# 360CVGroup/PlanGen

Hardware: AMD Instinct MI355X
Metric: images/sec, 384px layout2image (576 image tokens, CFG, VQ-16 decode), bs=64 per MI355X (higher is better)
Workload: dtype bf16

## Files before the change

plangen_amd/csrc/attn_decode.h:

```cpp
#pragma once
#include <type_traits>
#include "kernels.h"

template <int NV>
__device__ __forceinline__ void sum_slabs(const float* __restrict__ p, long slab, int S, const int (&offs)[NV], float (&acc)[NV]) {
    for (int s0 = 0; s0 < S; s0 += 4) {
        float t[4][NV];
#pragma unroll
        for (int u = 0; u < 4; ++u) {
            const float* q = p + (long)(s0 + u < S ? s0 + u : S - 1) * slab;
#pragma unroll
            for (int v = 0; v < NV; ++v) t[u][v] = q[offs[v]];
        }
#pragma unroll
        for (int u = 0; u < 4; ++u)
            if (s0 + u < S) {
#pragma unroll
                for (int v = 0; v < NV; ++v) acc[v] += t[u][v];
            }
    }
}

template <typename T, int UN, int NW, int ABL = 0>
__global__ __launch_bounds__(64 * NW) void attn_decode_fused_kernel(const int32_t* __restrict__ row_order, const int32_t* __restrict__ len_p,
                                                              const int32_t* __restrict__ n_dec_p, T* __restrict__ kc, T* __restrict__ vc,
                                                              int nh, int slots, int shared_len, int shared_row,
                                                              const float* __restrict__ qkv, long slab, T* __restrict__ obuf,
                                                              const float* __restrict__ cos_t, const float* __restrict__ sin_t,
                                                              const int32_t* __restrict__ pos_off_p, int S, int max_pos, float scale) {
    constexpr int EPV = ET<T>::EPV, LPK = 128 / EPV, KPI = 64 / LPK, NST = NW * KPI;
    __shared__ float s_o[NST][128];
    __shared__ float s_m[NST], s_l[NST];
    __shared__ __attribute__((aligned(16))) float s_q[128];
    __shared__ float s_k[128], s_v[128];
    __shared__ float s_new;
    constexpr int NIT = (ABL & 32) ? 2 : 1;
    const int tid = threadIdx.x, w = tid >> 6, l = tid & 63;
    const int head = blockIdx.x;
// ... 24 lines not shown
            kv[u] = NTL ? __builtin_nontemporal_load((const u32x4*)(kb + (long)key * 128)) : *(const u32x4*)(kb + (long)key * 128);
        }
#pragma unroll
        for (int u = 0; u < UN; ++u) {
            int key = base + u * KPI + grp;
            key = key < k1 ? key : k1 - 1;
            key = key < 0 ? 0 : key;
            vv[u] = NTL ? __builtin_nontemporal_load((const u32x4*)(vb + (long)key * 128)) : *(const u32x4*)(vb + (long)key * 128);
        }
    };
    const int seg_k1 = sh ? kstart : nprev;
    const int base0 = w * KPW;
    const bool have0 = base0 < seg_k1;
    const int o6[6] = {0, 64, HD, HD + 64, 2 * HD, 2 * HD + 64};
    float t4[4][6], cs = 0.f, sn = 0.f;
    int pos = pos_off_p[row] + slot;
    if (pos >= max_pos) pos = max_pos - 1;
    const float* const qrow = qkv + (long)row * 3 * HD + head * 128 + (tid & 63);
    if (tid < 64) {
        if constexpr (ABL & 2) {
#pragma unroll
            for (int u = 0; u < 4; ++u)
#pragma unroll
                for (int v = 0; v < 6; ++v) t4[u][v] = 0.01f * (float)(tid + v);
            cs = 1.f; sn = 0.f;
        } else {
#pragma unroll
        for (int u = 0; u < 4; ++u) {
            const float* qq = qrow + (long)(u < S ? u : S - 1) * slab;
#pragma unroll
            for (int v = 0; v < 6; ++v) t4[u][v] = qq[o6[v]];
        }
        cs = cos_t[(long)pos * 64 + tid]; sn = sin_t[(long)pos * 64 + tid];
        }
    }
    __builtin_amdgcn_sched_barrier(0);
    if (sh) issue(kshr, vshr, base0, seg_k1, std::false_type{}); else issue(kpriv, vpriv, base0, seg_k1, std::true_type{});
    __builtin_amdgcn_sched_barrier(0);

    if (tid < 64) {
        const int j = tid;
        float a6[6] = {0.f, 0.f, 0.f, 0.f, 0.f, 0.f};
#pragma unroll
        for (int u = 0; u < 4; ++u)
#pragma unroll
            for (int v = 0; v < 6; ++v) asm volatile("" : "+v"(t4[u][v])::"memory");
#pragma unroll
        for (int u = 0; u < 4; ++u)
            if (u < S) {
#pragma unroll
                for (int v = 0; v < 6; ++v) a6[v] += t4[u][v];
            }
        if (S > 4) sum_slabs<6>(qrow + 4 * slab, slab, S - 4, o6, a6);
        const float q0 = a6[0], q1 = a6[1], k0 = a6[2], k1 = a6[3], v0 = a6[4], v1 = a6[5];
        const float c = cs;
// ... 125 lines not shown
    __syncthreads();
    if (tid < 128) {
        float Mx = s_new;
#pragma unroll
        for (int i = 0; i < NST; ++i) Mx = fmaxf(Mx, s_m[i]);
        const float fn = __expf(s_new - Mx);
        float num = fn * s_v[tid], den = fn;
#pragma unroll
        for (int i = 0; i < NST; ++i) {
            const float f = (s_m[i] > -INFINITY) ? __expf(s_m[i] - Mx) : 0.f;
            num = fmaf(f, s_o[i][tid], num);
            den = fmaf(f, s_l[i], den);
        }
        ET<T>::st(obuf + (long)row * HD + head * 128 + tid, num / den);
    }
    if (!(ABL & 1) && tid < 64 && slot < slots) {
        const float* src = (l < 32 ? s_k : s_v) + (l & 31) * 4;
        T* dst = (l < 32 ? kc : vc) + cbase + (long)slot * 128 + (l & 31) * 4;
        if constexpr (sizeof(T) == 2) {
            u32x2 pk; pk.x = pack_bf16x2(src[0], src[1]); pk.y = pack_bf16x2(src[2], src[3]);
            *(u32x2*)dst = pk;
        } else {
            *(f32x4*)dst = *(const f32x4*)src;
        }
    }
    if constexpr (NIT > 1) __syncthreads();
    }
}
```

plangen_amd/csrc/diag_api.hip:

```cpp
#include "engine.h"
#include "diag.h"

extern "C" {

int pg_diag_set_option(pg_handle h, const char* key, int64_t value) {
    if (!h || !key) return PG_ERR_ARG;
    h->tune.diag = diag_hooks();
    if (!strcmp(key, "skip_attn")) { h->skip_attn = value != 0; return PG_OK; }
    if (!strcmp(key, "attn_variant")) { h->tune.attn_variant = (int)value; h->tune_epoch++; return PG_OK; }
    if (!strcmp(key, "attn_waves")) { h->tune.attn_waves = (int)value; h->tune_epoch++; return PG_OK; }
    if (!strcmp(key, "split_target_small")) { h->tune.split_small = (int)value; h->tune_epoch++; return PG_OK; }
    if (!strcmp(key, "split_target_mid")) { h->tune.split_mid = (int)value; h->tune_epoch++; return PG_OK; }
    if (!strcmp(key, "gn_epilogue256")) { h->tune.gn_epilogue256 = value != 0; return PG_OK; }
    if (!strcmp(key, "defer_norm")) { h->defer_norm = value != 0; h->tune_epoch++; return PG_OK; }
    if (!strcmp(key, "fuse_rope")) { h->fuse_rope = value != 0; h->tune_epoch++; return PG_OK; }
    if (!strcmp(key, "force_swiglu")) { h->force_swiglu = value != 0; h->tune_epoch++; return PG_OK; }
    if (!strcmp(key, "lpt_order")) { h->lpt_order = value != 0; h->tune_epoch++; return PG_OK; }
    h->err = std::string("unknown diagnostics option ") + key;
    return PG_ERR_ARG;
}

}
```

plangen_amd/csrc/diag_ops.hip:

```cpp
#include <type_traits>
#include <vector>
#include "kernels.h"
#include "diag.h"
#include "../../include/plangen_hip.h"

namespace {
struct LocalTune {
    PgTune t;
    const PgTune* saved;
    LocalTune() : saved(pg_tune) { t.diag = nullptr; pg_tune = &t; }
    ~LocalTune() { pg_tune = saved; }
};
constexpr int kMaxGridYZ = 65535;
bool to_host(std::vector<int32_t>& dst, const int32_t* src, int n) {
    dst.assign(n > 0 ? n : 0, 0);
    if (n <= 0) return true;
    if (!src) return false;
    return hipMemcpy(dst.data(), src, (size_t)n * 4, hipMemcpyDeviceToHost) == hipSuccess;
}
int launched(hipStream_t s) { (void)s; return hipGetLastError() == hipSuccess ? PG_OK : PG_ERR_HIP; }
}

extern "C" {

// ... 30 lines not shown
    }
    void* q = qbuf;
    if (!q && hipMalloc(&q, (size_t)M * nh * 128 * (is_bf16 ? 2 : 4)) != hipSuccess) return PG_ERR_HIP;
    if (is_bf16) {
        launch_rope_kv<bf16>(s, qkv, S, slab, (bf16*)q, (bf16*)kc, (bf16*)vc, cos_t, sin_t, st, 0, M, nh, slots, max_pos);
        launch_attn<bf16>(s, (const bf16*)q, (bf16*)obuf, (const bf16*)kc, (const bf16*)vc, st, 0, M, nh, slots, scale);
    } else {
        launch_rope_kv<float>(s, qkv, S, slab, (float*)q, (float*)kc, (float*)vc, cos_t, sin_t, st, 0, M, nh, slots, max_pos);
        launch_attn<float>(s, (const float*)q, (float*)obuf, (const float*)kc, (const float*)vc, st, 0, M, nh, slots, scale);
    }
    const int rc = launched(s);
    if (!qbuf) { (void)hipStreamSynchronize(s); (void)hipFree(q); }
    return rc;
}

int pg_diag_op_attn_prefill(int is_bf16, int path, const void* qbuf, void* obuf, const void* kc, const void* vc, const int32_t* row_off,
                            const int32_t* len, const int32_t* tok_row, const int32_t* tok_j, int R, int max_len, int Ntok, int nh, int slots,
                            float scale, pg_stream stream) {
    if (!qbuf || !obuf || !kc || !vc || !row_off || !len || !tok_row || !tok_j) return PG_ERR_ARG;
    if (path < 0 || path > 2 || (path > 0 && !is_bf16)) return PG_ERR_ARG;
    if (R < 1 || R > kMaxGridYZ || nh < 1 || nh > kMaxGridYZ || Ntok < 1 || Ntok > 0x7fffffff / 8 || max_len < 1 || max_len > slots) return PG_ERR_ARG;
    std::vector<int32_t> hoff, hlen, hrow, hj;
    if (!to_host(hoff, row_off, R) || !to_host(hlen, len, R) || !to_host(hrow, tok_row, Ntok) || !to_host(hj, tok_j, Ntok)) return PG_ERR_HIP;
    for (int m = 0; m < Ntok; ++m)
        if (hrow[m] < 0 || hrow[m] >= R || hj[m] < 0 || hj[m] >= slots) return PG_ERR_ARG;
    for (int r = 0; r < R; ++r) {
        if (hlen[r] < 0 || hlen[r] > max_len) return PG_ERR_ARG;
        if (hoff[r] < 0) continue;
        if (hlen[r] < 1 || (long)hoff[r] + hlen[r] > Ntok) return PG_ERR_ARG;
        for (int j = 0; j < hlen[r]; ++j)
// ... 28 lines not shown
```

plangen_amd/csrc/engine.h:

```cpp
#pragma once
#include <hip/hip_runtime.h>
#include <math.h>
#include <stdio.h>
#include <stdlib.h>
#include <string.h>

#include <algorithm>
#include <map>
#include <string>
#include <type_traits>
#include <vector>

#include "../../include/plangen_hip.h"
#include "kernels.h"

#define HIPCHK(expr)                                                                                     \
    do {                                                                                                 \
        hipError_t _e = (expr);                                                                          \
        if (_e != hipSuccess) {                                                                          \
            char _b[512];                                                                                \
            snprintf(_b, sizeof _b, "%s:%d %s -> %s", __FILE__, __LINE__, #expr, hipGetErrorString(_e)); \
            this->err = _b;                                                                              \
            return PG_ERR_HIP;                                                                           \
        }                                                                                                \
// ... 26 lines not shown
struct LinW { void* w = nullptr; float* b = nullptr; int out = 0, in = 0; };
struct VitBlockW { NormW n1, n2; LinW qkv, proj, fc1, fc2; };
struct VqNet { ConvW conv_in; ResBlockW mid0, mid2; AttnW mid1; std::vector<VqLevel> levels; NormW norm_out; ConvW conv_out; };

struct pg_engine {
    pg_config cfg{};
    int dev = 0;
    bool bf = true;
    size_t esz = 2;
    std::string err;
    std::vector<void*> allocs;
    int64_t bytes = 0;
    std::map<std::string, Slot> slots_map;

    struct Layer { void *wqkv, *wo, *wgu, *wd, *ln1, *ln2; void *wqkv_t = nullptr, *wo_t = nullptr, *wgu_t = nullptr, *wd_t = nullptr;
                   void* wqkv_p = nullptr; };
    void *gh_w1_t = nullptr, *gh_w2_t = nullptr, *lm_head_t = nullptr;
    int tile_one(hipStream_t s, const void* src, void** dst, int N, int K);
    std::vector<Layer> layers;
    void* norm_w = nullptr; float* embed = nullptr; void* lm_head = nullptr;
    void *gh_w1 = nullptr, *gh_w2 = nullptr; float *gh_b1 = nullptr, *gh_b2 = nullptr;
    float *ge_w = nullptr, *al_w0 = nullptr, *al_b0 = nullptr, *al_w2 = nullptr, *al_b2 = nullptr;
    float* gen_table = nullptr;
    float *codebook = nullptr, *codebook_n = nullptr, *pq_w = nullptr, *pq_b = nullptr;
    void* pq_table = nullptr;
    void* qc_w = nullptr; float* qc_b = nullptr;
    float *enc_in_w = nullptr, *enc_in_b = nullptr;
    VqNet dec, enc;
    LinW vit_patch, al0, al2; float* vit_pos = nullptr; std::vector<VitBlockW> vit_blocks; NormW vit_norm;
    float* vx = nullptr; void *vt = nullptr, *vqk = nullptr, *vvt = nullptr, *vo = nullptr, *vh = nullptr, *vp = nullptr, *val = nullptr;
    float* vscore = nullptr;
// ... 11 lines not shown
    int32_t* h_stage2[2] = {nullptr, nullptr};
    hipEvent_t ev_stage[2] = {nullptr, nullptr}; bool stage_used[2] = {false, false}; int stage_sel = 0;
    int32_t* d_flag = nullptr; int32_t* h_flag = nullptr;
    float* cfg_pv = nullptr; int* cfg_pi = nullptr;
    float* txt_mix = nullptr;
    float* cfg_mix = nullptr;
    SampleParams* d_sparams = nullptr; TextParams* d_tparams = nullptr;
    int32_t *d_out_tok = nullptr, *d_force_tok = nullptr; uint8_t* d_force_mask = nullptr; int64_t* d_text_out = nullptr;
    int rng_image_offset = 0;
    PgTune tune;
    int tune_epoch = 0;
    void* kv = nullptr;
    long max_tok = 0;
    float* x = nullptr; void* xn = nullptr; float* part = nullptr; long part_elems = 0, decode_part_elems = 0;
    float* ssq_part = nullptr;
    bool defer_norm = true;
    void *qbuf = nullptr, *obuf = nullptr, *hbuf = nullptr, *hfin = nullptr, *gh_in = nullptr, *gh_mid = nullptr;
    void* vbuf[4] = {nullptr, nullptr, nullptr, nullptr}; long vbuf_elems = 0;
    void *cur = nullptr, *t1 = nullptr, *t2 = nullptr, *t3 = nullptr;
    void *aq = nullptr, *ak = nullptr, *avt = nullptr, *ao = nullptr, *ap = nullptr; float* ascore = nullptr;
    float *gn_stats = nullptr, *gn_ws = nullptr, *gn_coef = nullptr;
    const void* gn_part_of = nullptr; int gn_part_n = 0, gn_part_b = 0;
    float* enc_z = nullptr;
    void* stage_dev = nullptr; long stage_bytes = 0;
    hipStream_t istream = nullptr; hipEvent_t ev_in = nullptr, ev_out = nullptr;
    hipEvent_t ev_t0 = nullptr, ev_t1 = nullptr, ev_p0 = nullptr, ev_p1 = nullptr, ev_v0 = nullptr, ev_v1 = nullptr;
    hipGraphExec_t gexec = nullptr; std::vector<int64_t> gkey;
    hipGraphExec_t gexec_txt = nullptr; std::vector<int64_t> gkey_txt;
    void drop_graphs() { if (gexec) { (void)hipGraphExecDestroy(gexec); gexec = nullptr; } if (gexec_txt) { (void)hipGraphExecDestroy(gexec_txt); gexec_txt = nullptr; } }
    bool use_graph = false;
// ... 95 lines not shown
```

plangen_amd/csrc/engine_core.hip:

```cpp
#include "engine.h"

void pg_engine::add_slot(const std::string& name, void* dst, SlotKind k, long n, int a, int b, int c) {
    Slot s; s.dst = dst; s.kind = k; s.n = n; s.a = a; s.b = b; s.c = c;
    slots_map[name] = s;
}
int pg_engine::alloc_conv(const std::string& name, ConvW& cw, int cout, int cin, int k) {
    cw.cin = cin; cw.cout = cout; cw.k = k;
    TRY(dalloc(&cw.w, (size_t)cout * cin * k * k * esz));
    TRY(dalloc(&cw.b, (size_t)cout * 4));
    add_slot(name + ".weight", cw.w, k == 1 ? K_T : K_CONV, (long)cout * cin * k * k, cout, cin, k * k);
    slot_shape(name + ".weight", {cout, cin, k, k});
    add_slot(name + ".bias", cw.b, K_F32, cout);
    return PG_OK;
}
int pg_engine::alloc_norm(const std::string& name, NormW& nw, int c) {
    nw.c = c;
    TRY(dalloc(&nw.g, (size_t)c * 4));
    TRY(dalloc(&nw.b, (size_t)c * 4));
    add_slot(name + ".weight", nw.g, K_F32, c);
    add_slot(name + ".bias", nw.b, K_F32, c);
    return PG_OK;
}
int pg_engine::alloc_res(const std::string& name, ResBlockW& r, int cin, int cout) {
    TRY(alloc_norm(name + ".norm1", r.n1, cin));
// ... 422 lines not shown
    }
    {
        std::vector<float> c((size_t)max_pos * 64), sn((size_t)max_pos * 64);
        for (int j = 0; j < 64; ++j) {
            const float inv = 1.0f / powf(cfg.rope_theta, (float)(2 * j) / 128.0f);
            for (int p = 0; p < max_pos; ++p) {
                const float f = (float)p * inv;
                c[(size_t)p * 64 + j] = cosf(f); sn[(size_t)p * 64 + j] = sinf(f);
            }
        }
        HIPCHK(hipMemcpy(cos_t, c.data(), c.size() * 4, hipMemcpyHostToDevice));
        HIPCHK(hipMemcpy(sin_t, sn.data(), sn.size() * 4, hipMemcpyHostToDevice));
    }
    if (bf) {
        const int Hh2 = H(), I = cfg.inter, HDm = HD();
        for (Layer& ly : layers) {
            TRY(tile_one(s, ly.wqkv, &ly.wqkv_t, 3 * HDm, Hh2));
            const long max_packed = (long)cfg.max_rows * cfg.max_prompt;
            const bool can_fuse = ((max_packed + 255) / 256) * ((3L * HDm + 255) / 256) >= 200;
            if ((Hh2 & 7) == 0 && can_fuse) {
                if (!ly.wqkv_p) TRY(dalloc(&ly.wqkv_p, (size_t)3 * HDm * Hh2 * 2));
                launch_interleave_qk(s, (const bf16*)ly.wqkv, (bf16*)ly.wqkv_p, cfg.n_heads, Hh2);
            }
            TRY(tile_one(s, ly.wo, &ly.wo_t, Hh2, HDm));
            TRY(tile_one(s, ly.wgu, &ly.wgu_t, 2 * I, Hh2));
            TRY(tile_one(s, ly.wd, &ly.wd_t, Hh2, I));
        }
        TRY(tile_one(s, gh_w1, &gh_w1_t, cfg.gen_head_dim, Hh2));
        TRY(tile_one(s, gh_w2, &gh_w2_t, cfg.img_vocab, cfg.gen_head_dim));
        if (lm_head) TRY(tile_one(s, lm_head, &lm_head_t, cfg.vocab, Hh2));
        HIPCHK(hipStreamSynchronize(s));
    }
    HIPCHK(hipGetLastError());
    finalized = miss == 0 || allow_partial;
    return PG_OK;
}
int pg_engine::tile_one(hipStream_t s, const void* src, void** dst, int N, int K) {
    if ((N & 15) || (K % 128)) { *dst = nullptr; return PG_OK; }
    if (!*dst) TRY(dalloc(dst, (size_t)N * K * 2));
    launch_tile_weights(s, (const bf16*)src, (bf16*)*dst, N, K);
    return PG_OK;
}
```

plangen_amd/csrc/engine_llm.hip:

```cpp
#include "engine.h"

template <typename T>
void pg_engine::gemm_llm(hipStream_t s, const T* a, const T* W, int M, int N, int K, bool allow_skinny, const void* Wt) {
    slab_last = (long)M * N;
    if constexpr (std::is_same<T, bf16>::value) {
        if (allow_skinny && M <= 512 && K % 128 == 0) {
            const int S = skinny_pick_splits(N, K, M);
            if ((long)S * M * N <= part_elems) {
                launch_gemm_skinny(s, a, W, part, M, N, K, S, (const bf16*)Wt);
                S_last = S;
                return;
            }
        }
    }
    GemmA ga; ga.ptr = a; ga.lda = K;
    GemmEpi e; e.out = part; e.out_f32 = 1; e.ldc = N;
    launch_gemm<T>(s, ga, W, K, 0, e, M, N, K, 1);
    S_last = 1;
}

template <typename T>
void pg_engine::gemm_residual(hipStream_t s, const T* a, const T* W, int M, int N, int K) {
    GemmA ga; ga.ptr = a; ga.lda = K;
    GemmEpi e; e.out = x; e.out_f32 = 1; e.ldc = N; e.residual = x; e.res_f32 = 1;
// ... 2 lines not shown
}

template <typename T>
void pg_engine::run_layers(hipStream_t s, int M, int mode, T* final_out, int32_t* advance) {
    const int Hh = H(), I = cfg.inter, HDm = HD();
    const bool sk = mode == 0;
    int S_pend = 0; long slab_pend = 0;
    const float scale = 1.0f / sqrtf(128.0f);
    tc_on = time_attn && mode == 0 && (n_dec_host % (time_stride > 0 ? time_stride : 1)) == 0;
    const double wb = (double)esz;
    auto norm_bytes = [&](int S) { return (double)M * Hh * (4.0 * (S + 2) + wb); };
    for (int li = 0; li < cfg.n_layers; ++li) {
        const Layer& ly = layers[li];
        tic(s); toc(s, TC_EMPTY, 0.0);
        tic(s);
        bool d1 = false, d2 = false;
        int Sq = 0;
        if constexpr (std::is_same<T, bf16>::value) {
            if (sk && defer_norm && Hh == 2048 && S_pend > 0 && S_pend <= 8 && slab_pend <= 0x7fffffffL && ly.wqkv_t) {
                Sq = skinny_pick_splits(3 * HDm, Hh, M);
                d1 = deferred_norm_ok(M, 3 * HDm, Hh, Sq) && (long)Sq * M * 3 * HDm <= part_elems;
            }
            if (d1) launch_rmsnorm_defer(s, x, part, S_pend, slab_pend, (const bf16*)ly.ln1, (bf16*)xn, ssq_part, M, Hh);
        }
        if (!d1) launch_rmsnorm<T>(s, x, part, S_pend, slab_pend, (const T*)ly.ln1, (T*)xn, M, Hh, cfg.rms_eps);
        toc(s, TC_NORM, norm_bytes(S_pend));
        tic(s);
        bool qkv_fused = false;
        if constexpr (std::is_same<T, bf16>::value) {
            if (mode == 1 && prefill_rope_epi && ly.wqkv_p) {
                GemmA ga; ga.ptr = xn; ga.lda = Hh;
                GemmEpi ge; ge.act = 3; ge.out = qbuf; ge.out_f32 = 0; ge.ldc = 3 * HDm;
                ge.rope.qbuf = qbuf; ge.rope.kc = kc(li); ge.rope.vc = vc(li); ge.rope.cos_t = cos_t; ge.rope.sin_t = sin_t;
                ge.rope.tok_row = d_tok_row; ge.rope.tok_j = d_tok_j; ge.rope.pos_off = d_pos_off;
                ge.rope.nh = cfg.n_heads; ge.rope.slots = slots; ge.rope.max_pos = max_pos;
                qkv_fused = gemm256_try(s, ga, (const bf16*)ly.wqkv_p, Hh, 0, ge, M, 3 * HDm, Hh, 1, 1, 0);
            }
        }
        if constexpr (std::is_same<T, bf16>::value) {
            if (d1) {
                d1 = launch_gemm_skinny_deferred(s, (const bf16*)xn, (const bf16*)ly.wqkv_t, part, M, 3 * HDm, Hh, Sq, ssq_part, cfg.rms_eps);
                if (d1) { S_last = Sq; slab_last = (long)M * 3 * HDm; qkv_fused = true; }
                else launch_rmsnorm<T>(s, x, part, 0, 0, (const T*)ly.ln1, (T*)xn, M, Hh, cfg.rms_eps);
            }
        }
        if (!qkv_fused) gemm_llm<T>(s, (const T*)xn, (const T*)ly.wqkv, M, 3 * HDm, Hh, sk, ly.wqkv_t);
        toc(s, TC_QKV, 3.0 * HDm * Hh * wb);
        if (mode == 0 && skip_attn) {
        } else if (mode == 0 && fuse_rope) {
            tic(s);
            launch_attn_decode_fused<T>(s, part, S_last, slab_last, (T*)obuf, (T*)kc(li), (T*)vc(li), cos_t, sin_t, seq(), M,
                                        cfg.n_heads, slots, max_pos, scale);
        } else {
            if (!qkv_fused)
                launch_rope_kv<T>(s, part, S_last, slab_last, (T*)qbuf, (T*)kc(li), (T*)vc(li), cos_t, sin_t, seq(), mode, M,
                                  cfg.n_heads, slots, max_pos);
            tic(s);
            bool done = false;
            if constexpr (std::is_same<T, bf16>::value) {
                if (mode == 1 && flash_prefill) {
                    launch_attn_prefill_flash(s, (const bf16*)qbuf, (bf16*)obuf, (const bf16*)kc(li), (const bf16*)vc(li), d_row_off, d_len,
                                              R, max_len_host, cfg.n_heads, slots, scale);
                    done = true;
// ... 378 lines not shown
```

plangen_amd/csrc/gemm.hip:

```cpp
#include "kernels.h"

#include "gemm_common.h"
#include <type_traits>

#define BIG_BM 128
#define BIG_BN 128
#define BIG_BK 64
#define BIG_TILE_BYTES (128 * 64 * 2)
#define BIG_LDS (4 * BIG_TILE_BYTES)

template <class AL, class EP>
__global__ __launch_bounds__(256, 2) void gemm_big_kernel(AL al, const bf16* __restrict__ W, long ldb,
                                                         long strideA, long strideB, long strideA2, long strideB2, EP ep,
                                                         int M, int N, int K, int ntm, int ntn) {
    extern __shared__ __attribute__((aligned(16))) char smem[];
    const int tid = threadIdx.x, w = tid >> 6, l = tid & 63;
    const int batch = blockIdx.y, batch2 = blockIdx.z;
    const long coff = (long)batch * ep.e.strideC + (long)batch2 * ep.e.strideC2;
    const long roff = (long)batch * ep.e.strideR;
    const int t = xcd_remap(blockIdx.x, gridDim.x);
    int tile_m, tile_n;
    if (((ntm | ntn) & 7) == 0) {
        const int sup = t >> 6, in = t & 63, gm = ntm >> 3;
        tile_m = (sup % gm) * 8 + (in & 7);
// ... 296 lines not shown
bool deferred_norm_ok(int M, int N, int K, int S) {
    if (K != 2048) return false;
    const int sg = pg_tune->stream_gemm >= 0 ? pg_tune->stream_gemm : (M > 64 ? 2 : 15);
    const int nck = S > 0 ? K / SK_BK / S : 0;
    return M > 64 && M <= 128 && N >= 4096 && (N % 128) == 0 && !(sg & 1) && !(sg & 4) && S > 0 && nck * S * SK_BK == K
           && (nck == 1 || nck == 2 || nck == 4 || nck == 8 || nck == 16);
}
bool launch_gemm_skinny_deferred(hipStream_t s, const bf16* xw, const bf16* Wt, float* out, int M, int N, int K, int S, const float* ssq, float eps) {
    if (!Wt || !ssq || !deferred_norm_ok(M, N, K, S)) return false;
    return sk3_prod_tiled<0, true>(s, xw, Wt, out, M, N, K, S, SkRowScale{ssq, eps});
}
bool launch_gemm_skinny_swiglu_deferred(hipStream_t s, const bf16* xw, const bf16* Wt, bf16* h, int M, int N, int K, const float* ssq, float eps) {
    if (!Wt || !ssq || !deferred_norm_ok(M, N, K, 1)) return false;
    return sk3_prod_tiled<1, true>(s, xw, Wt, (float*)h, M, N, K, 1, SkRowScale{ssq, eps});
}
void launch_gemm_skinny(hipStream_t s, const bf16* x, const bf16* W, float* out, int M, int N, int K, int S, const bf16* Wt) {
    if (M <= 0) return;
    if (sk4_prod<4>(s, x, Wt, out, M, N, K, S)) return;
    if (Wt && sk3_prod_tiled<0, true>(s, x, Wt, out, M, N, K, S)) return;
    if (!sk3_prod<0>(s, x, W, out, M, N, K, S)) launch_gemm_skinny_v1(s, x, W, out, M, N, K, S);
}
bool launch_gemm_skinny_tiled_only(hipStream_t s, const bf16* x, const bf16* Wt, float* out, int M, int N, int K, int S) {
    return sk4_prod<4>(s, x, Wt, out, M, N, K, S) || sk3_prod_tiled<0, true>(s, x, Wt, out, M, N, K, S);
}
bool launch_gemm_skinny_swiglu(hipStream_t s, const bf16* x, const bf16* W, bf16* h, int M, int N, int K, const bf16* Wt) {
    if (M <= 0) return true;
    if (sk4_prod<3>(s, x, Wt, (float*)h, M, N, K, 1)) return true;
    if (Wt && sk3_prod_tiled<1, true>(s, x, Wt, (float*)h, M, N, K, 1)) return true;
    return sk3_prod<1>(s, x, W, (float*)h, M, N, K, 1);
}
// ... 1 lines not shown
```

plangen_amd/csrc/gemm_skinny.h:

```cpp
#pragma once
#include "kernels.h"
#include "gemm_common.h"

#define SK_BK 128
#define SK_ROWB 288


template <int MT, int NW>
__device__ __forceinline__ void skinny_store_tile(char* smem, const f32x4 (&acc)[MT], float* __restrict__ o, int M, int N,
                                                  int mbase, int nbase, int w, int g, int lr, int tid, const float* rs = nullptr) {
    constexpr int LD = NW * 16 + 4, NTH = NW * 64, V4 = NW * 4;
    float* t = (float*)smem;
    __syncthreads();
#pragma unroll
    for (int mt = 0; mt < MT; ++mt)
#pragma unroll
        for (int r = 0; r < 4; ++r) t[(mt * 16 + g * 4 + r) * LD + w * 16 + lr] = acc[mt][r];
    __syncthreads();
    for (int v = tid; v < MT * 16 * V4; v += NTH) {
        const int row = v / V4, c4 = (v % V4) * 4;
        const int m = mbase + row, n = nbase + c4;
        if (m < M && n < N) {
            f32x4 v4 = *(const f32x4*)(t + row * LD + c4);
            if (rs) { const float r_ = rs[row]; v4.x *= r_; v4.y *= r_; v4.z *= r_; v4.w *= r_; }
// ... 239 lines not shown


template <int MT, int EPI, int NW = 4, bool TILED = false, int D = 2>
static bool sk3_prod_nck(hipStream_t s, const bf16* x, const bf16* W, float* out, int M, int N, int K, int S, int nck, SkRowScale rsc = {}) {
    switch (nck) {
        case 1: launch_sk3<MT, 1, D, true, EPI, NW, TILED>(s, x, W, out, M, N, K, S, rsc); return true;
        case 2: launch_sk3<MT, 2, D, true, EPI, NW, TILED>(s, x, W, out, M, N, K, S, rsc); return true;
        case 4: launch_sk3<MT, 4, D, true, EPI, NW, TILED>(s, x, W, out, M, N, K, S, rsc); return true;
        case 8: launch_sk3<MT, 8, D, true, EPI, NW, TILED>(s, x, W, out, M, N, K, S, rsc); return true;
        case 11: launch_sk3<MT, 11, D, true, EPI, NW, TILED>(s, x, W, out, M, N, K, S, rsc); return true;
        case 16: launch_sk3<MT, 16, D, true, EPI, NW, TILED>(s, x, W, out, M, N, K, S, rsc); return true;
        case 22: launch_sk3<MT, 22, D, true, EPI, NW, TILED>(s, x, W, out, M, N, K, S, rsc); return true;
        default: return false;
    }
}
constexpr int sk4_wait_count(int c, int NCK, int XD, int WD, int MT, int ahead = 0) {
    int ops = 0, lastX[64] = {};
    for (int p = 0; p < XD - 1 && p < NCK; ++p) { ops += MT; lastX[p] = ops; }
    for (int p = 0; p < WD && p < NCK; ++p) ops += 4;
    for (int it = 0; it < NCK; ++it) {
        if (it == c) return ops - lastX[(c + ahead < NCK) ? c + ahead : NCK - 1];
        if (it + XD - 1 < NCK) { ops += MT; lastX[it + XD - 1] = ops; }
        if (it + WD < NCK) ops += 4;
    }
    return 0;
}
constexpr int sk4_wait_count_w(int c, int NCK, int XD, int WD, int MT) {
    int ops = 0, lastW[64] = {};
    for (int p = 0; p < XD - 1 && p < NCK; ++p) ops += MT;
    for (int p = 0; p < WD && p < NCK; ++p) { ops += 4; lastW[p] = ops; }
// ... 287 lines not shown
```

plangen_amd/csrc/kernels.h:

```cpp
#pragma once
#include <hip/hip_runtime.h>
#include <stdint.h>
#include "common.h"

struct PgTune {
    int split_small = 128, split_mid = 256, split_big = 128;
    int gemm256 = 1;
    int conv_halo = 1;
    int attn_waves = 0;
    int attn_variant = 0;
    int prefill_attn = 2;
    int gn_epilogue256 = 0;
    int vq_tail_fused = 0;
    int vq_argmin_multi = 1;
    int vit_attn = 2;
    int ln_wave = 1;
    int stream_gemm = -1;
    const struct PgDiagHooks* diag = nullptr;
};
struct SeqState; struct GemmA; struct GemmEpi;
struct PgDiagHooks {
    bool (*attn_decode)(hipStream_t s, bool is_bf16, const float* qkv, int S, long slab, void* obuf, void* kc, void* vc, const float* cos_t, const float* sin_t,
                        const SeqState& st, int M, int nh, int slots, int max_pos, float scale);
    bool (*gemm_big_wave)(hipStream_t s, const GemmA& a, const bf16* W, long ldb, const GemmEpi& e, int M, int N, int K, int batch, int batch2);
// ... 42 lines not shown
                   int* gn_nsplit = nullptr);
void launch_gn_finalize(hipStream_t s, const float* ws, float* stats, float* coef, const float* gamma, const float* beta, int B,
                        int nsplit, int HW, int C, float eps);
bool conv_out_halo_try(hipStream_t s, const bf16* x, const bf16* w, const float* bias, const bf16* zeros, void* out, int out_bf16,
                       int B, int H, int Wd, int Cin, int Cout);
bool conv_out_gn_try(hipStream_t s, const float* x_f32, const float* coef, const bf16* w, const float* bias, void* out, int out_bf16,
                     int B, int H, int Wd, int Cin, int Cout, int swish);

int skinny_pick_splits(int N, int K);
int skinny_pick_splits(int N, int K, int M);
bool launch_gemm_skinny_swiglu(hipStream_t s, const bf16* x, const bf16* W, bf16* h, int M, int N, int K, const bf16* Wt = nullptr);
void launch_gemm_skinny(hipStream_t s, const bf16* x, const bf16* W, float* out, int M, int N, int K, int S, const bf16* Wt = nullptr);
bool deferred_norm_ok(int M, int N, int K, int S);
bool launch_gemm_skinny_deferred(hipStream_t s, const bf16* xw, const bf16* Wt, float* out, int M, int N, int K, int S, const float* ssq, float eps);
bool launch_gemm_skinny_swiglu_deferred(hipStream_t s, const bf16* xw, const bf16* Wt, bf16* h, int M, int N, int K, const float* ssq, float eps);
void launch_rmsnorm_defer(hipStream_t s, float* x, const float* partial, int S, long slab, const bf16* w, bf16* xw, float* ssq, int M, int H);
void launch_tile_weights(hipStream_t s, const bf16* src, bf16* dst, int N, int K);
void launch_interleave_qk(hipStream_t s, const bf16* src, bf16* dst, int nh, int K);

template <typename T>
void launch_rmsnorm(hipStream_t s, float* x, const float* partial, int S, long slab, const T* w, T* xn,
                    int M, int H, float eps, int32_t* advance = nullptr);

void launch_embed_gather(hipStream_t s, const float* table, const int32_t* ids, const int32_t* src_idx, float* dst,
                         int n, int H, int vocab);
void launch_copy_rows(hipStream_t s, const void* src, const int32_t* src_idx, void* dst, const int32_t* dst_idx,
                      int n, long row_bytes);
void launch_rows_to_f32(hipStream_t s, const void* src, int src_bf16, const int32_t* src_row, float* dst, int n, int H);
void launch_f32_to_rows(hipStream_t s, const float* src, void* dst, int dst_bf16, const int32_t* dst_row, int n, int H);
template <typename T>
// ... 10 lines not shown
    const int32_t* row_order;
};
template <typename T>
void launch_rope_kv(hipStream_t s, const float* qkv, int S, long slab, T* qbuf, T* kc, T* vc,
                    const float* cos_t, const float* sin_t, SeqState st, int mode, int M, int nh,
                    int slots, int max_pos);
template <typename T>
void launch_attn(hipStream_t s, const T* qbuf, T* obuf, const T* kc, const T* vc, SeqState st, int mode,
                 int M, int nh, int slots, float scale);
void launch_attn_prefill_flash(hipStream_t s, const bf16* qbuf, bf16* obuf, const bf16* kc, const bf16* vc,
                               const int32_t* row_off, const int32_t* len, int R, int max_len, int nh, int slots, float scale);
template <typename T>
void launch_attn_decode_fused(hipStream_t s, const float* qkv, int S, long slab, T* obuf, T* kc, T* vc,
                              const float* cos_t, const float* sin_t, SeqState st, int M, int nh, int slots,
                              int max_pos, float scale);
template <typename T>
void launch_silu_mul(hipStream_t s, const float* gu, int S, long slab, T* h, int M, int I);
template <typename T>
void launch_bias_act(hipStream_t s, const float* partial, int S, long slab, const float* bias, T* out,
                     int M, int N, int act);
void launch_bias_f32(hipStream_t s, const float* partial, int S, long slab, const float* bias, float* out, int M, int N);

struct SampleParams { float cfg_weight, temperature; uint64_t seed; int32_t T, has_force, has_mask, img_off; int32_t top_k; float top_p; };
struct SampleArgs {
    const float* logits_partial; int S; long slab; const float* bias; int V;
    const SampleParams* p;
    const int32_t* force_tok; const uint8_t* force_mask;
    int32_t* out_tok;
    float* logits_out;
    const float* embed_table;
// ... 77 lines not shown
```

plangen_amd/csrc/llm_kernels.hip:

```cpp
#include <cstdlib>
#include <type_traits>
#include "kernels.h"
#include "attn_decode.h"


template <typename T, int NV, int SB = 4>
__global__ __launch_bounds__(256) void rmsnorm_kernel(float* __restrict__ x, const float* __restrict__ partial,
                                                     int S, long slab, const T* __restrict__ w,
                                                     T* __restrict__ xn, int H, float eps, int32_t* __restrict__ advance) {
    __shared__ float red[4];
    rmsnorm_row<T, NV, false, SB>(blockIdx.x, x, partial, S, slab, w, xn, H, eps, red);
    if (advance && blockIdx.x == 0 && threadIdx.x == 0) *advance += 1;
}
template <typename T, int SB>
__global__ __launch_bounds__(512) void rmsnorm512_kernel(float* __restrict__ x, const float* __restrict__ partial, const T* __restrict__ w,
                                                        T* __restrict__ xn, int32_t* __restrict__ advance, int S, int slab, int H, float eps) {
    __shared__ float red[8];
    rmsnorm_row<T, 1, false, SB, 512>(blockIdx.x, x, partial, S, (long)slab, w, xn, H, eps, red);
    if (advance && blockIdx.x == 0 && threadIdx.x == 0) *advance += 1;
}
template <typename T>
void launch_rmsnorm(hipStream_t s, float* x, const float* partial, int S, long slab, const T* w, T* xn,
                    int M, int H, float eps, int32_t* advance) {
    if (M <= 0) return;
// ... 247 lines not shown
void launch_attn_decode_fused(hipStream_t s, const float* qkv, int S, long slab, T* obuf, T* kc, T* vc,
                              const float* cos_t, const float* sin_t, SeqState st, int M, int nh, int slots,
                              int max_pos, float scale) {
    if (M <= 0) return;
    if (pg_tune->diag && pg_tune->diag->attn_decode && pg_tune->diag->attn_decode(s, std::is_same<T, bf16>::value, qkv, S, slab, obuf, kc, vc, cos_t, sin_t, st, M, nh, slots, max_pos, scale)) return;
#define ATT_LAUNCH(U, W, A) hipLaunchKernelGGL((attn_decode_fused_kernel<T, U, W, A>), dim3(nh, M), dim3(64 * W), 0, s, st.row_order, st.len, st.n_dec, kc, vc, nh, slots, st.shared_len, st.shared_row, qkv, slab, obuf, cos_t, sin_t, st.pos_off, S, max_pos, scale)
    const bool small = (M * nh <= 512 && pg_tune->attn_waves != 4) || pg_tune->attn_waves == 8;
    if (small) ATT_LAUNCH(5, 8, 16);
    else ATT_LAUNCH(6, 4, 16);
#undef ATT_LAUNCH
}
template void launch_attn_decode_fused<float>(hipStream_t, const float*, int, long, float*, float*, float*, const float*, const float*, SeqState, int, int, int, int, float);
template void launch_attn_decode_fused<bf16>(hipStream_t, const float*, int, long, bf16*, bf16*, bf16*, const float*, const float*, SeqState, int, int, int, int, float);

template <typename T>
void launch_attn(hipStream_t s, const T* qbuf, T* obuf, const T* kc, const T* vc, SeqState st, int mode,
                 int M, int nh, int slots, float scale) {
    if (M <= 0) return;
    dim3 grid(M, nh), block(256);
    if (mode == 0) hipLaunchKernelGGL((attn_kernel<T, 8, true>), grid, block, 0, s, qbuf, obuf, kc, vc, st, mode, nh, slots, scale);
    else hipLaunchKernelGGL((attn_kernel<T, 8, false>), grid, block, 0, s, qbuf, obuf, kc, vc, st, mode, nh, slots, scale);
}
template void launch_attn<float>(hipStream_t, const float*, float*, const float*, const float*, SeqState, int, int, int, int, float);
template void launch_attn<bf16>(hipStream_t, const bf16*, bf16*, const bf16*, const bf16*, SeqState, int, int, int, int, float);

template <typename T>
__global__ void silu_mul_kernel(const float* __restrict__ gu, int S, long slab, T* __restrict__ h, int I) {
    const int m = blockIdx.y;
    const int n = blockIdx.x * blockDim.x + threadIdx.x;
    if (n >= I) return;
// ... 812 lines not shown
```

Baseline: 37.42.

## Fuse RoPE and KV-cache write into skinny QKV GEMM epilogue for decode

Adds a skinny QKV GEMM variant whose epilogue applies the deferred RMS norm scale, combines the two K-split partials, applies rotary embedding, and writes Q to a bf16 buffer and K/V directly into the cache. It uses pre-tiled, QK-interleaved weights built at finalize time. The decode attention kernel gets a mode that reads these precomputed bf16 Q/K/V instead of summing fp32 split partials and redoing RoPE. The goal is to cut fp32 partial-slab traffic and per-head RoPE work in attention, at the cost of extra weight memory and a path limited to 64<M<=128 rows with hidden size 2048.

```diff
diff --git a/plangen_amd/csrc/attn_decode.h b/plangen_amd/csrc/attn_decode.h
--- a/plangen_amd/csrc/attn_decode.h
+++ b/plangen_amd/csrc/attn_decode.h
@@ -21,7 +21,7 @@
     }
 }
 
-template <typename T, int UN, int NW, int ABL = 0>
+template <typename T, int UN, int NW, int ABL = 0, bool QKB = false>
 __global__ __launch_bounds__(64 * NW) void attn_decode_fused_kernel(const int32_t* __restrict__ row_order, const int32_t* __restrict__ len_p,
                                                               const int32_t* __restrict__ n_dec_p, T* __restrict__ kc, T* __restrict__ vc,
                                                               int nh, int slots, int shared_len, int shared_row,
@@ -76,11 +76,21 @@
     const bool have0 = base0 < seg_k1;
     const int o6[6] = {0, 64, HD, HD + 64, 2 * HD, 2 * HD + 64};
     float t4[4][6], cs = 0.f, sn = 0.f;
-    int pos = pos_off_p[row] + slot;
+    int pos = QKB ? 0 : pos_off_p[row] + slot;
     if (pos >= max_pos) pos = max_pos - 1;
     const float* const qrow = qkv + (long)row * 3 * HD + head * 128 + (tid & 63);
+    uint32_t raw[6] = {0u, 0u, 0u, 0u, 0u, 0u};
     if (tid < 64) {
-        if constexpr (ABL & 2) {
+        if constexpr (QKB) {
+            const T* const qp = (const T*)qkv + (long)row * HD + head * 128 + tid;
+            const T* const kp = kc + cbase + (long)nprev * 128 + tid; const T* const vp = vc + cbase + (long)nprev * 128 + tid;
+            const T* const src[6] = {qp, qp + 64, kp, kp + 64, vp, vp + 64};
+#pragma unroll
+            for (int v = 0; v < 6; ++v) {
+                if constexpr (sizeof(T) == 2) raw[v] = *(const uint16_t*)src[v];
+                else raw[v] = __float_as_uint(*(const float*)src[v]);
+            }
+        } else if constexpr (ABL & 2) {
 #pragma unroll
             for (int u = 0; u < 4; ++u)
 #pragma unroll
@@ -100,7 +110,18 @@
     if (sh) issue(kshr, vshr, base0, seg_k1, std::false_type{}); else issue(kpriv, vpriv, base0, seg_k1, std::true_type{});
     __builtin_amdgcn_sched_barrier(0);
 
-    if (tid < 64) {
+    if (QKB && tid < 64) {
+        const int j = tid;
+        float f6[6];
+#pragma unroll
+        for (int v = 0; v < 6; ++v) {
+            asm volatile("" : "+v"(raw[v])::"memory");
+            f6[v] = __uint_as_float(sizeof(T) == 2 ? raw[v] << 16 : raw[v]);
+        }
+        s_q[j] = f6[0] * scale; s_q[j + 64] = f6[1] * scale;
+        s_k[j] = f6[2]; s_k[j + 64] = f6[3]; s_v[j] = f6[4]; s_v[j + 64] = f6[5];
+    }
+    if (!QKB && tid < 64) {
         const int j = tid;
         float a6[6] = {0.f, 0.f, 0.f, 0.f, 0.f, 0.f};
 #pragma unroll
@@ -256,7 +277,7 @@
         }
         ET<T>::st(obuf + (long)row * HD + head * 128 + tid, num / den);
     }
-    if (!(ABL & 1) && tid < 64 && slot < slots) {
+    if (!QKB && !(ABL & 1) && tid < 64 && slot < slots) {
         const float* src = (l < 32 ? s_k : s_v) + (l & 31) * 4;
         T* dst = (l < 32 ? kc : vc) + cbase + (long)slot * 128 + (l & 31) * 4;
         if constexpr (sizeof(T) == 2) {
diff --git a/plangen_amd/csrc/diag_api.hip b/plangen_amd/csrc/diag_api.hip
--- a/plangen_amd/csrc/diag_api.hip
+++ b/plangen_amd/csrc/diag_api.hip
@@ -13,6 +13,10 @@
     if (!strcmp(key, "split_target_mid")) { h->tune.split_mid = (int)value; h->tune_epoch++; return PG_OK; }
     if (!strcmp(key, "gn_epilogue256")) { h->tune.gn_epilogue256 = value != 0; return PG_OK; }
     if (!strcmp(key, "defer_norm")) { h->defer_norm = value != 0; h->tune_epoch++; return PG_OK; }
+    if (!strcmp(key, "decode_qkv_epi")) {
+        if (value != 0 && value != 2 && value != 4) return PG_ERR_ARG;
+        h->decode_qkv_epi = (int)value; h->tune_epoch++; return PG_OK;
+    }
     if (!strcmp(key, "fuse_rope")) { h->fuse_rope = value != 0; h->tune_epoch++; return PG_OK; }
     if (!strcmp(key, "force_swiglu")) { h->force_swiglu = value != 0; h->tune_epoch++; return PG_OK; }
     if (!strcmp(key, "lpt_order")) { h->lpt_order = value != 0; h->tune_epoch++; return PG_OK; }
diff --git a/plangen_amd/csrc/diag_ops.hip b/plangen_amd/csrc/diag_ops.hip
--- a/plangen_amd/csrc/diag_ops.hip
+++ b/plangen_amd/csrc/diag_ops.hip
@@ -68,6 +68,32 @@
     return rc;
 }
 
+int pg_diag_op_qkv_epi(const void* xw, const void* Wqkv, const float* ssq, float eps, void* qbuf, void* kc, void* vc, const float* cos_t,
+                       const float* sin_t, const int32_t* len, const int32_t* pos_off, const int32_t* n_dec, int M, int nh, int K, int slots,
+                       int max_pos, int geom, pg_stream stream) {
+    if (!xw || !Wqkv || !ssq || !qbuf || !kc || !vc || !cos_t || !sin_t || !len || !pos_off || !n_dec) return PG_ERR_ARG;
+    if (nh < 1 || nh > 64 || slots < 1 || max_pos < 1) return PG_ERR_ARG;
+    LocalTune lt;
+    if (!decode_qkv_epi_ok(M, nh, K, geom)) return PG_ERR_ARG;
+    std::vector<int32_t> hl, hn, hp;
+    if (!to_host(hl, len, M) || !to_host(hn, n_dec, 1) || !to_host(hp, pos_off, M)) return PG_ERR_HIP;
+    for (int r = 0; r < M; ++r)
+        if (hl[r] < 0 || hn[0] < 0 || (long)hl[r] + hn[0] >= slots || hp[r] < 0) return PG_ERR_ARG;
+    const hipStream_t s = (hipStream_t)stream;
+    const size_t wb = (size_t)3 * nh * 128 * K * 2;
+    void *wi = nullptr, *wt = nullptr;
+    if (hipMalloc(&wi, wb) != hipSuccess) return PG_ERR_HIP;
+    if (hipMalloc(&wt, wb) != hipSuccess) { (void)hipFree(wi); return PG_ERR_HIP; }
+    launch_interleave_qk(s, (const bf16*)Wqkv, (bf16*)wi, nh, K);
+    launch_tile_weights(s, (const bf16*)wi, (bf16*)wt, 3 * nh * 128, K);
+    const SkQkvEpi qe{(bf16*)qbuf, (bf16*)kc, (bf16*)vc, cos_t, sin_t, len, pos_off, n_dec, nh, slots, max_pos};
+    const bool ok = launch_gemm_skinny_qkv_epi(s, (const bf16*)xw, (const bf16*)wt, ssq, eps, qe, M, K, geom);
+    const int rc = ok ? launched(s) : PG_ERR_ARG;
+    (void)hipStreamSynchronize(s);
+    (void)hipFree(wi); (void)hipFree(wt);
+    return rc;
+}
+
 int pg_diag_op_attn_prefill(int is_bf16, int path, const void* qbuf, void* obuf, const void* kc, const void* vc, const int32_t* row_off,
                             const int32_t* len, const int32_t* tok_row, const int32_t* tok_j, int R, int max_len, int Ntok, int nh, int slots,
                             float scale, pg_stream stream) {
diff --git a/plangen_amd/csrc/engine.h b/plangen_amd/csrc/engine.h
--- a/plangen_amd/csrc/engine.h
+++ b/plangen_amd/csrc/engine.h
@@ -64,7 +64,8 @@
     std::map<std::string, Slot> slots_map;
 
     struct Layer { void *wqkv, *wo, *wgu, *wd, *ln1, *ln2; void *wqkv_t = nullptr, *wo_t = nullptr, *wgu_t = nullptr, *wd_t = nullptr;
-                   void* wqkv_p = nullptr; };
+                   void* wqkv_p = nullptr;
+                   void* wqkv_pt = nullptr; };
     void *gh_w1_t = nullptr, *gh_w2_t = nullptr, *lm_head_t = nullptr;
     int tile_one(hipStream_t s, const void* src, void** dst, int N, int K);
     std::vector<Layer> layers;
@@ -106,6 +107,7 @@
     long max_tok = 0;
     float* x = nullptr; void* xn = nullptr; float* part = nullptr; long part_elems = 0, decode_part_elems = 0;
     float* ssq_part = nullptr;
+    int decode_qkv_epi = 2;
     bool defer_norm = true;
     void *qbuf = nullptr, *obuf = nullptr, *hbuf = nullptr, *hfin = nullptr, *gh_in = nullptr, *gh_mid = nullptr;
     void* vbuf[4] = {nullptr, nullptr, nullptr, nullptr}; long vbuf_elems = 0;
diff --git a/plangen_amd/csrc/engine_core.hip b/plangen_amd/csrc/engine_core.hip
--- a/plangen_amd/csrc/engine_core.hip
+++ b/plangen_amd/csrc/engine_core.hip
@@ -460,6 +460,7 @@
     }
     if (bf) {
         const int Hh2 = H(), I = cfg.inter, HDm = HD();
+        void* qk_tmp = nullptr;
         for (Layer& ly : layers) {
             TRY(tile_one(s, ly.wqkv, &ly.wqkv_t, 3 * HDm, Hh2));
             const long max_packed = (long)cfg.max_rows * cfg.max_prompt;
@@ -468,6 +469,15 @@
                 if (!ly.wqkv_p) TRY(dalloc(&ly.wqkv_p, (size_t)3 * HDm * Hh2 * 2));
                 launch_interleave_qk(s, (const bf16*)ly.wqkv, (bf16*)ly.wqkv_p, cfg.n_heads, Hh2);
             }
+            if (Hh2 == 2048 && cfg.head_dim == 128 && cfg.max_rows > 64) {
+                const void* inter = ly.wqkv_p;
+                if (!inter) {
+                    if (!qk_tmp) HIPCHK(hipMalloc(&qk_tmp, (size_t)3 * HDm * Hh2 * 2));
+                    launch_interleave_qk(s, (const bf16*)ly.wqkv, (bf16*)qk_tmp, cfg.n_heads, Hh2);
+                    inter = qk_tmp;
+                }
+                TRY(tile_one(s, inter, &ly.wqkv_pt, 3 * HDm, Hh2));
+            }
             TRY(tile_one(s, ly.wo, &ly.wo_t, Hh2, HDm));
             TRY(tile_one(s, ly.wgu, &ly.wgu_t, 2 * I, Hh2));
             TRY(tile_one(s, ly.wd, &ly.wd_t, Hh2, I));
@@ -476,6 +486,7 @@
         TRY(tile_one(s, gh_w2, &gh_w2_t, cfg.img_vocab, cfg.gen_head_dim));
         if (lm_head) TRY(tile_one(s, lm_head, &lm_head_t, cfg.vocab, Hh2));
         HIPCHK(hipStreamSynchronize(s));
+        if (qk_tmp) HIPCHK(hipFree(qk_tmp));
     }
     HIPCHK(hipGetLastError());
     finalized = miss == 0 || allow_partial;
diff --git a/plangen_amd/csrc/engine_llm.hip b/plangen_amd/csrc/engine_llm.hip
--- a/plangen_amd/csrc/engine_llm.hip
+++ b/plangen_amd/csrc/engine_llm.hip
@@ -40,12 +40,14 @@
         const Layer& ly = layers[li];
         tic(s); toc(s, TC_EMPTY, 0.0);
         tic(s);
-        bool d1 = false, d2 = false;
+        bool d1 = false, d2 = false, qk_epi = false;
         int Sq = 0;
         if constexpr (std::is_same<T, bf16>::value) {
             if (sk && defer_norm && Hh == 2048 && S_pend > 0 && S_pend <= 8 && slab_pend <= 0x7fffffffL && ly.wqkv_t) {
                 Sq = skinny_pick_splits(3 * HDm, Hh, M);
                 d1 = deferred_norm_ok(M, 3 * HDm, Hh, Sq) && (long)Sq * M * 3 * HDm <= part_elems;
+                qk_epi = d1 && Sq == 2 && decode_qkv_epi > 0 && fuse_rope && !skip_attn && ly.wqkv_pt && !(tune.diag && tune.attn_variant)
+                         && decode_qkv_epi_ok(M, cfg.n_heads, Hh, decode_qkv_epi);
             }
             if (d1) launch_rmsnorm_defer(s, x, part, S_pend, slab_pend, (const bf16*)ly.ln1, (bf16*)xn, ssq_part, M, Hh);
         }
@@ -64,7 +66,13 @@
             }
         }
         if constexpr (std::is_same<T, bf16>::value) {
-            if (d1) {
+            if (qk_epi) {
+                const SeqState st = seq();
+                const SkQkvEpi qe{(bf16*)qbuf, (bf16*)kc(li), (bf16*)vc(li), cos_t, sin_t, st.len, st.pos_off, st.n_dec, cfg.n_heads, slots, max_pos};
+                qk_epi = launch_gemm_skinny_qkv_epi(s, (const bf16*)xn, (const bf16*)ly.wqkv_pt, ssq_part, cfg.rms_eps, qe, M, Hh, decode_qkv_epi);
+                if (qk_epi) { S_last = 0; slab_last = (long)M * 3 * HDm; qkv_fused = true; }
+            }
+            if (d1 && !qk_epi) {
                 d1 = launch_gemm_skinny_deferred(s, (const bf16*)xn, (const bf16*)ly.wqkv_t, part, M, 3 * HDm, Hh, Sq, ssq_part, cfg.rms_eps);
                 if (d1) { S_last = Sq; slab_last = (long)M * 3 * HDm; qkv_fused = true; }
                 else launch_rmsnorm<T>(s, x, part, 0, 0, (const T*)ly.ln1, (T*)xn, M, Hh, cfg.rms_eps);
@@ -73,6 +81,10 @@
         if (!qkv_fused) gemm_llm<T>(s, (const T*)xn, (const T*)ly.wqkv, M, 3 * HDm, Hh, sk, ly.wqkv_t);
         toc(s, TC_QKV, 3.0 * HDm * Hh * wb);
         if (mode == 0 && skip_attn) {
+        } else if (mode == 0 && qk_epi) {
+            tic(s);
+            if constexpr (std::is_same<T, bf16>::value)
+                launch_attn_decode_qk<bf16>(s, (const bf16*)qbuf, (bf16*)obuf, (bf16*)kc(li), (bf16*)vc(li), seq(), M, cfg.n_heads, slots, scale);
         } else if (mode == 0 && fuse_rope) {
             tic(s);
             launch_attn_decode_fused<T>(s, part, S_last, slab_last, (T*)obuf, (T*)kc(li), (T*)vc(li), cos_t, sin_t, seq(), M,
diff --git a/plangen_amd/csrc/gemm.hip b/plangen_amd/csrc/gemm.hip
--- a/plangen_amd/csrc/gemm.hip
+++ b/plangen_amd/csrc/gemm.hip
@@ -334,6 +334,15 @@
     if (!Wt || !ssq || !deferred_norm_ok(M, N, K, 1)) return false;
     return sk3_prod_tiled<1, true>(s, xw, Wt, (float*)h, M, N, K, 1, SkRowScale{ssq, eps});
 }
+bool decode_qkv_epi_ok(int M, int nh, int K, int geom) {
+    return K == 2048 && M > 64 && M <= 128 && nh > 0 && (geom == 2 || geom == 4) && deferred_norm_ok(M, 3 * nh * 128, K, 2);
+}
+bool launch_gemm_skinny_qkv_epi(hipStream_t s, const bf16* xw, const bf16* Wpt, const float* ssq, float eps, const SkQkvEpi& ep, int M, int K, int geom) {
+    if (!Wpt || !ssq || !ep.qbuf || !ep.kc || !ep.vc || !decode_qkv_epi_ok(M, ep.nh, K, geom)) return false;
+    if (geom == 2) launch_skq<4, 8, 2, 4, 2>(s, xw, Wpt, ssq, eps, ep, M, K);
+    else launch_skq<4, 8, 2, 4, 1>(s, xw, Wpt, ssq, eps, ep, M, K);
+    return true;
+}
 void launch_gemm_skinny(hipStream_t s, const bf16* x, const bf16* W, float* out, int M, int N, int K, int S, const bf16* Wt) {
     if (M <= 0) return;
     if (sk4_prod<4>(s, x, Wt, out, M, N, K, S)) return;
diff --git a/plangen_amd/csrc/gemm_skinny.h b/plangen_amd/csrc/gemm_skinny.h
--- a/plangen_amd/csrc/gemm_skinny.h
+++ b/plangen_amd/csrc/gemm_skinny.h
@@ -277,6 +277,139 @@
         default: return false;
     }
 }
+constexpr int skq_main_lds(int MT, int NW, int KG) {
+    const int XL = KG * 2 * MT * 16 * SK_ROWB, TL = 2 * MT * 16 * (NW * 16 + 4) * 4;
+    return XL > TL ? XL : TL;
+}
+template <int MT, int NCK, int D, int NW, int KG>
+__global__ __launch_bounds__(64 * NW * KG, (NW * KG >= 8 ? 1 : 2)) void gemm_skinny_qkv_kernel(const bf16* __restrict__ x, const bf16* __restrict__ W,
+                                                                                          const float* __restrict__ ssq, SkQkvEpi ep, int M, int K, float eps) {
+    extern __shared__ __attribute__((aligned(16))) char smem[];
+    constexpr int XB = MT * 16 * SK_ROWB, NTG = 64 * NW, NTH = NTG * KG, BN = 16 * NW, NCG = 2 * NCK / KG, NA = 2 / KG;
+    constexpr int LD = BN + 4, TF = MT * 16 * LD;
+    constexpr int RS_OFF = skq_main_lds(MT, NW, KG);
+    constexpr int XV = MT * 256 / NTG;
+    static_assert((MT * 256) % NTG == 0 && (KG == 1 || KG == 2) && 128 % BN == 0, "tile must divide over the wave group; a block stays inside one head");
+    const int tid = threadIdx.x, w = tid >> 6, l = tid & 63, g = l >> 4, lr = l & 15;
+    const int kg = w / NW, wn = w - kg * NW, gt = tid - kg * NTG;
+    const int mbase = blockIdx.y * (MT * 16), bx = blockIdx.x;
+    const bf16* wp = W + ((long)(bx * NW + wn) * (K / SK_BK) + kg * NCG) * 2048 + l * 8;
+    const bf16* xp = x + kg * NCG * SK_BK;
+    char* const xsm = smem + kg * 2 * XB;
+
+    u32x4 xs[XV];
+    auto xload = [&](int c) {
+#pragma unroll
+        for (int j = 0; j < XV; ++j) {
+            const int v = gt + j * NTG, row = v >> 4, cv = v & 15;
+            const int m = mbase + row;
+            xs[j] = *(const u32x4*)(xp + (long)(m < M ? m : M - 1) * K + c * SK_BK + cv * 8);
+        }
+    };
+    auto xstore = [&](int buf) {
+#pragma unroll
+        for (int j = 0; j < XV; ++j) {
+            const int v = gt + j * NTG, row = v >> 4, cv = v & 15;
+            *(u32x4*)(xsm + buf * XB + row * SK_ROWB + cv * 16) = xs[j];
+        }
+    };
+    bf16x8 wr[D][4];
+#pragma unroll
+    for (int c = 0; c < D && c < NCG; ++c)
+#pragma unroll
+        for (int i = 0; i < 4; ++i) wr[c][i] = *(const bf16x8*)(wp + c * 2048 + i * 512);
+    f32x4 acc[NA][MT];
+#pragma unroll
+    for (int a = 0; a < NA; ++a)
+#pragma unroll
+        for (int i = 0; i < MT; ++i) acc[a][i] = (f32x4){0.f, 0.f, 0.f, 0.f};
+    xload(0);
+    float* const rs = (float*)(smem + RS_OFF);
+    int* const s_pos = (int*)(smem + RS_OFF) + MT * 16;
+    int* const s_slot = s_pos + MT * 16;
+    if (tid < MT * 16) {
+        const int m = mbase + tid, mc = m < M ? m : M - 1;
+        const float* pp = ssq + (long)mc * 8;
+        const f32x4 a = *(const f32x4*)pp, b = *(const f32x4*)(pp + 4);
+        rs[tid] = rsqrtf((((a.x + a.y) + (a.z + a.w)) + ((b.x + b.y) + (b.z + b.w))) / (float)K + eps);
+        const int slot = ep.len[mc] + *ep.n_dec;
+        const int pos = ep.pos_off[mc] + slot;
+        s_pos[tid] = pos < ep.max_pos ? pos : ep.max_pos - 1;
+        s_slot[tid] = slot < ep.slots ? slot : ep.slots - 1;
+    }
+    xstore(0);
+    __syncthreads();
+#pragma unroll
+    for (int c = 0; c < NCG; ++c) {
+        if (c + 1 < NCG) xload(c + 1);
+        skinny_mfma_chunk<MT>(xsm + (c & 1) * XB, lr, g, wr[c % D], acc[c / NCK]);
+        if (c + D < NCG) {
+#pragma unroll
+            for (int i = 0; i < 4; ++i) wr[c % D][i] = *(const bf16x8*)(wp + (c + D) * 2048 + i * 512);
+        }
+        if (c + 1 < NCG) {
+            xstore((c + 1) & 1);
+            __syncthreads();
+        }
+    }
+    float* const t = (float*)smem;
+    __syncthreads();
+#pragma unroll
+    for (int a = 0; a < NA; ++a) {
+        float* const th = t + (KG == 2 ? kg : a) * TF;
+#pragma unroll
+        for (int mt = 0; mt < MT; ++mt)
+#pragma unroll
+            for (int r = 0; r < 4; ++r) {
+                const int row = mt * 16 + g * 4 + r;
+                th[row * LD + wn * 16 + lr] = __fmul_rn(acc[a][mt][r], rs[row]);
+            }
+    }
+    __syncthreads();
+    const int HDm = ep.nh * 128, nbase = bx * BN;
+    const int sec = nbase / HDm, hc = nbase - sec * HDm, head = hc >> 7, hc0 = hc & 127;
+    constexpr int IPR = BN / 8;
+    for (int v = tid; v < MT * 16 * IPR; v += NTH) {
+        const int row = v / IPR, u = v - row * IPR, tt = u >> 1, p4 = (u & 1) * 4;
+        const int m = mbase + row;
+        if (m >= M) continue;
+        const float* t0 = t + row * LD + tt * 16 + p4;
+        const f32x4 l0 = *(const f32x4*)t0, l1 = *(const f32x4*)(t0 + TF), h0 = *(const f32x4*)(t0 + 8), h1 = *(const f32x4*)(t0 + TF + 8);
+        float lo[4], hi[4];
+#pragma unroll
+        for (int e = 0; e < 4; ++e) { lo[e] = __fadd_rn(__fadd_rn(0.f, l0[e]), l1[e]); hi[e] = __fadd_rn(__fadd_rn(0.f, h0[e]), h1[e]); }
+        const long crow = (((long)m * ep.nh + head) * ep.slots + s_slot[row]) * 128;
+        u32x2 o0, o1;
+        bf16 *d0, *d1;
+        if (sec < 2) {
+            const int j = ((hc0 >> 4) + tt) * 8 + p4;
+            const f32x4 cs = *(const f32x4*)(ep.cos_t + (long)s_pos[row] * 64 + j), sn = *(const f32x4*)(ep.sin_t + (long)s_pos[row] * 64 + j);
+            float a[4], b[4];
+#pragma unroll
+            for (int e = 0; e < 4; ++e) { a[e] = rope_lo(lo[e], hi[e], cs[e], sn[e]); b[e] = rope_hi(lo[e], hi[e], cs[e], sn[e]); }
+            o0.x = pack_bf16x2(a[0], a[1]); o0.y = pack_bf16x2(a[2], a[3]);
+            o1.x = pack_bf16x2(b[0], b[1]); o1.y = pack_bf16x2(b[2], b[3]);
+            d0 = (sec == 0 ? ep.qbuf + (long)m * HDm + head * 128 : ep.kc + crow) + j;
+            d1 = d0 + 64;
+        } else {
+            o0.x = pack_bf16x2(lo[0], lo[1]); o0.y = pack_bf16x2(lo[2], lo[3]);
+            o1.x = pack_bf16x2(hi[0], hi[1]); o1.y = pack_bf16x2(hi[2], hi[3]);
+            d0 = ep.vc + crow + hc0 + tt * 16 + p4;
+            d1 = d0 + 8;
+        }
+        *(u32x2*)d0 = o0;
+        *(u32x2*)d1 = o1;
+    }
+}
+template <int MT, int NCK, int D, int NW, int KG>
+static void launch_skq(hipStream_t s, const bf16* x, const bf16* Wpt, const float* ssq, float eps, const SkQkvEpi& ep, int M, int K) {
+    constexpr int LDS = skq_main_lds(MT, NW, KG) + MT * 16 * 12;
+    auto kfn = gemm_skinny_qkv_kernel<MT, NCK, D, NW, KG>;
+    (void)PG_DYN_LDS(kfn, LDS);
+    dim3 grid(3 * ep.nh * 128 / (16 * NW), (M + MT * 16 - 1) / (MT * 16)), block(64 * NW * KG);
+    hipLaunchKernelGGL(kfn, grid, block, LDS, s, x, Wpt, ssq, ep, M, K, eps);
+}
+
 constexpr int sk4_wait_count(int c, int NCK, int XD, int WD, int MT, int ahead = 0) {
     int ops = 0, lastX[64] = {};
     for (int p = 0; p < XD - 1 && p < NCK; ++p) { ops += MT; lastX[p] = ops; }
diff --git a/plangen_amd/csrc/kernels.h b/plangen_amd/csrc/kernels.h
--- a/plangen_amd/csrc/kernels.h
+++ b/plangen_amd/csrc/kernels.h
@@ -80,6 +80,14 @@
 bool deferred_norm_ok(int M, int N, int K, int S);
 bool launch_gemm_skinny_deferred(hipStream_t s, const bf16* xw, const bf16* Wt, float* out, int M, int N, int K, int S, const float* ssq, float eps);
 bool launch_gemm_skinny_swiglu_deferred(hipStream_t s, const bf16* xw, const bf16* Wt, bf16* h, int M, int N, int K, const float* ssq, float eps);
+struct SkQkvEpi {
+    bf16* qbuf; bf16* kc; bf16* vc;
+    const float* cos_t; const float* sin_t;
+    const int32_t* len; const int32_t* pos_off; const int32_t* n_dec;
+    int nh, slots, max_pos;
+};
+bool decode_qkv_epi_ok(int M, int nh, int K, int geom);
+bool launch_gemm_skinny_qkv_epi(hipStream_t s, const bf16* xw, const bf16* Wpt, const float* ssq, float eps, const SkQkvEpi& ep, int M, int K, int geom);
 void launch_rmsnorm_defer(hipStream_t s, float* x, const float* partial, int S, long slab, const bf16* w, bf16* xw, float* ssq, int M, int H);
 void launch_tile_weights(hipStream_t s, const bf16* src, bf16* dst, int N, int K);
 void launch_interleave_qk(hipStream_t s, const bf16* src, bf16* dst, int nh, int K);
@@ -120,6 +128,8 @@
 void launch_attn_decode_fused(hipStream_t s, const float* qkv, int S, long slab, T* obuf, T* kc, T* vc,
                               const float* cos_t, const float* sin_t, SeqState st, int M, int nh, int slots,
                               int max_pos, float scale);
+template <typename T>
+void launch_attn_decode_qk(hipStream_t s, const T* qbuf, T* obuf, T* kc, T* vc, SeqState st, int M, int nh, int slots, float scale);
 template <typename T>
 void launch_silu_mul(hipStream_t s, const float* gu, int S, long slab, T* h, int M, int I);
 template <typename T>
diff --git a/plangen_amd/csrc/llm_kernels.hip b/plangen_amd/csrc/llm_kernels.hip
--- a/plangen_amd/csrc/llm_kernels.hip
+++ b/plangen_amd/csrc/llm_kernels.hip
@@ -285,6 +285,17 @@
 template void launch_attn_decode_fused<bf16>(hipStream_t, const float*, int, long, bf16*, bf16*, bf16*, const float*, const float*, SeqState, int, int, int, int, float);
 
 template <typename T>
+void launch_attn_decode_qk(hipStream_t s, const T* qbuf, T* obuf, T* kc, T* vc, SeqState st, int M, int nh, int slots, float scale) {
+    if (M <= 0) return;
+#define ATT_LAUNCH(U, W, A) hipLaunchKernelGGL((attn_decode_fused_kernel<T, U, W, A, true>), dim3(nh, M), dim3(64 * W), 0, s, st.row_order, st.len, st.n_dec, kc, vc, nh, slots, st.shared_len, st.shared_row, (const float*)qbuf, 0L, obuf, (const float*)nullptr, (const float*)nullptr, (const int32_t*)nullptr, 0, 1, scale)
+    const bool small = (M * nh <= 512 && pg_tune->attn_waves != 4) || pg_tune->attn_waves == 8;
+    if (small) ATT_LAUNCH(5, 8, 16);
+    else ATT_LAUNCH(6, 4, 16);
+#undef ATT_LAUNCH
+}
+template void launch_attn_decode_qk<bf16>(hipStream_t, const bf16*, bf16*, bf16*, bf16*, SeqState, int, int, int, float);
+
+template <typename T>
 void launch_attn(hipStream_t s, const T* qbuf, T* obuf, const T* kc, const T* vc, SeqState st, int mode,
                  int M, int nh, int slots, float scale) {
     if (M <= 0) return;
```

New measurement: 37.61 (median of 6 runs). No clear change (+0.5%).
